# jandrewrfarrell/RUFUS

Hardware: AMD Instinct MI355X
Metric: reads/sec through k-mer count+filter at k=25 (higher is better)
Workload: dtype u64; 1 GPU; synthetic 30x WGS trio (BASELINE configs[2]): genome 3100000000 bp, 620000000/620000000/620000000 x 150 bp reads per sample, on each of 1 GPU(s) 19 resident blocks of the subject (92 GB of packed reads in HBM, generated on the device in 3.3 s), 1000 SNVs, seed 12345, k=25, -s 8G -L 2, MinCov 5, MaxHashDepth 1200, MinQ 15, thresh 1; 2 minimizer-shard pass(es) per step (per-shard (pos,key)-sorted re; parallelism=read-block shard x1, mutant_kmers=24567, pulled_pairs=11560, passes=2, hbm_total=309220868096, hbm_free_at_start=308400881664, resident_read_bytes=92219805240, read_blocks=compact, run_map_budget_bytes=39836680704, checked=False, hbm_mapped_bytes=271656681472

## Files before the change

### include/rufus_hip.h

```cpp
#ifndef RUFUS_HIP_H
#define RUFUS_HIP_H

#include <stddef.h>
#include <stdint.h>

#ifdef __cplusplus
extern "C" {
#endif

#define RFX_OK 0
#define RFX_E_NODEVICE (-1)
#define RFX_E_INVAL (-2)
#define RFX_E_NOMEM (-3)
#define RFX_E_FULL (-4)
#define RFX_E_HIP (-5)
#define RFX_E_MIXEDCASE (-6)
#define RFX_E_RANGE (-7)
#define RFX_E_FORMAT (-8)

#define RFX_HISTO_BINS 10002

typedef struct rfx_ctx rfx_ctx;
typedef struct rfx_reads rfx_reads;
typedef struct rfx_table rfx_table;
// ... 166 lines not shown
const uint64_t* rfx_records_dev_pos(const rfx_records*);
int rfx_records_histo(const rfx_records*, uint64_t* histo );
int rfx_records_verify(const rfx_records*, uint32_t min_count, uint32_t max_count, uint64_t out[4]);
int rfx_records_checksum(const rfx_records*, uint64_t out[2]);
void rfx_records_free(rfx_records*);

int rfx_merge_unique(rfx_ctx*, const rfx_records* const* files, int n_files, uint32_t min_count, uint64_t* keys_out,
                     uint32_t* counts_out, uint64_t cap, uint64_t* n_out);
int rfx_query(const rfx_records* db, const uint64_t* keys, uint64_t n, uint32_t* counts_out);
int rfx_unique_to_subject(rfx_ctx*, const rfx_records* subject, const rfx_records* const* others, int n_others,
                          uint32_t min_count, uint32_t min_cov, uint32_t max_cov, uint64_t* keys_out,
                          uint32_t* counts_out, uint64_t cap, uint64_t* n_out);
rfx_records* rfx_records_subtract(rfx_ctx*, const rfx_records* a, const rfx_records* const* others, int n_others,
                                  uint32_t min_count, uint32_t max_count);

typedef struct rfx_binned rfx_binned;
typedef struct rfx_candidates rfx_candidates;
rfx_binned* rfx_count_finish_binned(rfx_table*, uint64_t lower, uint64_t upper, uint64_t* histo );
uint64_t rfx_binned_size(const rfx_binned*);
int rfx_binned_bits(const rfx_binned*);
void rfx_binned_free(rfx_binned*);
rfx_candidates* rfx_binned_strike(rfx_ctx*, rfx_binned* subject, const rfx_binned* control, uint32_t min_count,
                                  uint32_t max_count);
int rfx_candidates_strike(rfx_candidates*, const rfx_binned* control);
uint64_t rfx_candidates_size(const rfx_candidates*);
int rfx_candidates_get(const rfx_candidates*, uint64_t* keys_out);
int rfx_candidates_get_counts(const rfx_candidates*, uint32_t* counts_out);
int rfx_candidates_strike_records(rfx_candidates*, const rfx_records* exclude);
void rfx_candidates_free(rfx_candidates*);
int rfx_binned_get(const rfx_binned*, uint64_t* keys_out, uint32_t* counts_out, uint32_t* bins_out, uint64_t* at_out,
                   uint64_t cap, uint64_t* n_out);
int rfx_binned_checksum(const rfx_binned*, uint64_t out[2]);
int rfx_binned_verify(const rfx_binned*, uint64_t lower, uint64_t upper, uint64_t out[5]);
int rfx_binned_query(const rfx_binned*, const uint64_t* canonical_keys, uint64_t n, uint32_t* counts_out);
const uint64_t* rfx_binned_dev_keys(const rfx_binned*);
const uint32_t* rfx_binned_dev_counts(const rfx_binned*);

rfx_set* rfx_set_build(rfx_ctx*, const uint64_t* fwd_keys, uint64_t n, int k);
uint64_t rfx_set_size(const rfx_set*);
void rfx_set_free(rfx_set*);
int rfx_filter(rfx_set*, const rfx_reads*, int thresh, int last_base_skipped, uint32_t* hits_out,
               uint64_t* hitmask_out, uint64_t* n_hit_reads);
int rfx_filter_many(rfx_set*, const rfx_reads* const* blocks, int n, int thresh, int last_base_skipped,
                    uint64_t* const* hitmask_out, uint64_t* n_hit_reads);

#define RFX_SELECT_READS 0
// ... 32 lines not shown
```

### profiles/summarize_pmc.py

```python
#!/usr/bin/env python3
import collections
import csv
import json
import re
import sys


NOT_CHAIN = frozenset((
    "k_synth_reads", "k_copy16",
    "k_flag_absent", "k_flag_absent_tiled", "k_fa_bounds", "k_flag_gather", "k_flag_range", "k_flag_rank", "k_flag_present",
    "k_compact_count", "k_compact_scatter", "k_scan_u64", "k_query", "k_strike_bins", "k_strike_cands",
    "k_strike_query", "k_binned_sizes", "k_binned_scan", "k_binned_gather", "k_binned_checksum", "k_binned_verify", "k_binned_query",
    "k_filter", "k_filter_q", "k_filter_p", "k_filter_fast", "k_filter_big", "k_hits_mask", "k_mask_count", "k_set_bitmap",
    "k_set_bitmap_big", "k_set_bitmap_q", "k_set_bitmap_p",
    "k_set_insert", "k_set_bitmap_packed", "k_records_checksum", "k_records_verify", "k_check_sorted",
    "k_parse_records", "k_format_records", "k_txt_count", "k_txt_lines", "k_txt_reads", "k_txt_pack", "k_txt_nth", "k_bgzf_inflate", "k_reads_tile_count", "k_reads_tile_table", "k_reads_tile", "k_select_words", "k_select_table", "k_select_copy", "k_gather_sizes", "k_gather_table", "k_gather_copy", "k_compute_pos", "k_annotate", "k_overlap_pool", "k_overlap_score",
    "k_model_colsum", "k_model_dist", "k_model_rowtot", "k_model_sum", "k_model_terms", "k_model_weights",
))
CHAIN_KNOWN = frozenset((
    "k_msp_part1", "k_msp_replay", "k_msp_count", "k_col_sums", "k_bin_group_sums", "k_bin_offsets", "k_scan_tail", "k_scan_sums",
    "k_scan_apply", "k_part2", "k_flag_if_gt", "k_slice_tag", "k_bin_hist", "k_bin_hist_stamp", "k_bin_hist_multi", "k_msp_leaf",
    "k_surv_place", "k_surv_hist", "k_surv_sort", "k_histo_bins", "k_histo_staged", "k_bin_count", "k_part1", "k_leaf", "k_leaf_compact", "k_bin_scatter",
    "k_tmp_start", "k_split_bins", "k_coarse_counts", "k_histo", "k_count_reads", "k_count_pairs", "k_table_pairs", "k_tile_count",
    "k_tile_scan", "k_tile_emit",
))


def kname(s):
    m = re.search(r"(k_[a-z0-9_]+|__amd_rocclr_[A-Za-z]+)", s)
    return m.group(1) if m else s[:40]


def load(path, counter):
    agg = collections.defaultdict(lambda: [0, 0.0])
# ... 44 lines not shown
```

### rufus_amd/capi.py

```python
from __future__ import annotations

import ctypes as C
import os
import sys

import numpy as np

_HERE = os.path.dirname(os.path.abspath(__file__))
LIB_PATH = os.environ.get("RFX_LIB") or os.path.join(_HERE, "librufus_hip.so")

HISTO_BINS = 10002
PACK_COUNT, PACK_FILTER = 1, 2
COUNT_AUTO, COUNT_TABLE, COUNT_P2L, COUNT_MSP = 0, 1, 2, 3
E_FULL, E_RANGE, E_MIXEDCASE = -4, -7, -6
E_INVAL, E_FORMAT = -2, -8
SELECT_READS, SELECT_PAIRS = 0, 1

u8p, u32p, u64p = C.POINTER(C.c_uint8), C.POINTER(C.c_uint32), C.POINTER(C.c_uint64)

SIGNATURES = {
    "rfx_version": (C.c_char_p, []),
    "rfx_strerror": (C.c_char_p, [C.c_int]),
    "rfx_last_error": (C.c_char_p, []),
    "rfx_jf_matrix": (C.c_int, [C.c_int, C.c_int, u64p]),
# ... 8 lines not shown
    "rfx_open": (C.c_void_p, [C.c_int, C.c_size_t]),
    "rfx_close": (None, [C.c_void_p]),
    "rfx_sync": (C.c_int, [C.c_void_p]),
    "rfx_host_alloc": (C.c_void_p, [C.c_size_t]),
    "rfx_host_alloc_lazy": (C.c_void_p, [C.c_size_t]),
    "rfx_host_pin": (C.c_int, [C.c_void_p]),
    "rfx_host_cpus": (C.c_uint, []),
    "rfx_host_free": (None, [C.c_void_p]),
    "rfx_stream": (C.c_void_p, [C.c_void_p]),
    "rfx_mem_stats": (C.c_int, [C.c_void_p, u64p, u64p, u64p]),
    "rfx_memcpy_dev": (C.c_int, [C.c_void_p, C.c_void_p, C.c_void_p, C.c_size_t]),
    "rfx_prof_enable": (C.c_int, [C.c_void_p, C.c_int]),
    "rfx_prof_filter": (C.c_int, [C.c_void_p, C.c_char_p]),
    "rfx_prof_reset": (C.c_int, [C.c_void_p]),
    "rfx_prof_query": (C.c_int, [C.c_void_p, C.c_char_p, C.POINTER(C.c_double), u64p]),
    "rfx_prof_names": (C.c_int, [C.c_void_p, C.c_char_p, C.c_size_t]),
    "rfx_reads_device_bytes": (C.c_uint64, [C.c_void_p]),
    "rfx_records_subtract": (C.c_void_p, [C.c_void_p, C.c_void_p, C.POINTER(C.c_void_p), C.c_int, C.c_uint32, C.c_uint32]),
    "rfx_count_finish_binned": (C.c_void_p, [C.c_void_p, C.c_uint64, C.c_uint64, u64p]),
    "rfx_binned_size": (C.c_uint64, [C.c_void_p]),
    "rfx_binned_bits": (C.c_int, [C.c_void_p]),
    "rfx_binned_free": (None, [C.c_void_p]),
    "rfx_binned_strike": (C.c_void_p, [C.c_void_p, C.c_void_p, C.c_void_p, C.c_uint32, C.c_uint32]),
    "rfx_candidates_strike": (C.c_int, [C.c_void_p, C.c_void_p]),
    "rfx_candidates_size": (C.c_uint64, [C.c_void_p]),
    "rfx_candidates_get": (C.c_int, [C.c_void_p, u64p]),
    "rfx_candidates_free": (None, [C.c_void_p]),
    "rfx_candidates_get_counts": (C.c_int, [C.c_void_p, u32p]),
    "rfx_candidates_strike_records": (C.c_int, [C.c_void_p, C.c_void_p]),
    "rfx_binned_get": (C.c_int, [C.c_void_p, u64p, u32p, u32p, u64p, C.c_uint64, u64p]),
    "rfx_binned_checksum": (C.c_int, [C.c_void_p, u64p]),
    "rfx_binned_verify": (C.c_int, [C.c_void_p, C.c_uint64, C.c_uint64, u64p]),
    "rfx_binned_query": (C.c_int, [C.c_void_p, u64p, C.c_uint64, u32p]),
    "rfx_binned_dev_keys": (C.c_void_p, [C.c_void_p]),
    "rfx_binned_dev_counts": (C.c_void_p, [C.c_void_p]),
    "rfx_reads_upload": (C.c_void_p, [C.c_void_p, u64p, u32p, u32p, u32p, u32p, C.c_uint32]),
    "rfx_reads_free": (None, [C.c_void_p]),
    "rfx_reads_count": (C.c_uint32, [C.c_void_p]),
    "rfx_reads_bases": (C.c_uint64, [C.c_void_p]),
    "rfx_reads_words": (C.c_uint64, [C.c_void_p]),
    "rfx_reads_get": (C.c_int, [C.c_void_p, u64p, u32p, u32p, u32p, u32p]),
    "rfx_tile_plan": (C.c_int, [C.c_uint64, C.c_int, C.c_uint32, u64p, u32p]),
    "rfx_reads_tile": (C.c_void_p, [C.c_void_p, C.c_void_p, C.c_int, C.c_uint32]),
    "rfx_reads_select": (C.c_void_p, [C.c_void_p, C.c_void_p, u64p, C.c_int]),
    "rfx_reads_origin": (C.c_int, [C.c_void_p, u32p, u32p]),
    "rfx_filter_pull": (C.c_void_p, [C.c_void_p, C.POINTER(C.c_void_p), C.c_int, C.c_int, C.c_int, C.c_int, C.POINTER(u64p), u64p]),
# ... 825 lines not shown
        return k[k != np.uint64(0xFFFFFFFFFFFFFFFF)]

    def counts(self, raw_keys=None) -> np.ndarray:
        c = np.zeros(len(self), np.uint32)
        _check(lib().rfx_candidates_get_counts(self._h, _p(c, u32p)), "rfx_candidates_get_counts")
        k = self._raw_keys() if raw_keys is None else raw_keys
        return c[k != np.uint64(0xFFFFFFFFFFFFFFFF)]

    def keys_counts(self):
        k = self._raw_keys()
        return k[k != np.uint64(0xFFFFFFFFFFFFFFFF)], self.counts(k)

    def free(self):
        if self._h:
            lib().rfx_candidates_free(self._h)
            self._h = None


def binned_strike(ctx: Context, subject: Binned, control, min_count: int = 0, max_count: int = 0xFFFFFFFF) -> Candidates:
    return Candidates(ctx, lib().rfx_binned_strike(ctx._h, subject._h, control._h if control is not None else None,
                                                   min_count, max_count))


OVL_SAM, OVL_CONTIG, OVL_REGION = 0, 1, 2


def overlap_score(ctx: Context, a: bytes, cands, min_pct: float, min_ovl: int, variant: int = OVL_SAM) -> np.ndarray:
    nb = len(cands)
    arr = (C.c_char_p * max(nb, 1))(*cands)
    lens = (C.c_int * max(nb, 1))(*[len(x) for x in cands])
    out = np.zeros((max(nb, 1), 5), dtype=np.int32)
    _check(lib().rfx_overlap_score(ctx._h, a, len(a), arr, lens, nb, min_pct, min_ovl, variant,
                                   out.ctypes.data_as(C.POINTER(C.c_int))), "rfx_overlap_score")
    return out[:nb]


def model_residuals(ctx: Context, histo, cands, log_resid: bool, inflection: int, max_copy: int = 5) -> np.ndarray:
    histo = np.ascontiguousarray(histo, dtype=np.int64)
    cands = np.ascontiguousarray(cands, dtype=np.float64).reshape(-1, 5)
    out = np.zeros(len(cands), dtype=np.float64)
    _check(lib().rfx_model_residuals(ctx._h, _p(histo, C.POINTER(C.c_int64)), len(histo), cands.ctypes.data, len(cands),
                                     int(bool(log_resid)), inflection, max_copy, _p(out, C.POINTER(C.c_double))),
           "rfx_model_residuals")
    return out


# ... 71 lines not shown
```

### rufus_amd/csrc/rfx_api.hip

```cpp
#include <algorithm>
#include <condition_variable>
#include <mutex>
#include <cstdio>
#include <cstdlib>
#include <cstring>
#include <sys/mman.h>

#include <atomic>
#include <cerrno>
#include <chrono>
#include <queue>
#include <thread>
#include <vector>

#include <unistd.h>

#include "rfx_internal.h"

namespace {

thread_local char g_err[512] = "";

int hip_fail(hipError_t e, const char* what) {
  snprintf(g_err, sizeof g_err, "%s: %s", what, hipGetErrorString(e));
// ... 2882 lines not shown
void rfx_binned_free(rfx_binned* b) {
  if (!b) return;
  (void)hipSetDevice(b->ctx->device);
  leaf_stage_free(b->ctx, &b->st);
  dfree(b->ctx, b->bin_at);
  delete b;
}

rfx_candidates* rfx_binned_strike(rfx_ctx* c, rfx_binned* subject, const rfx_binned* control, uint32_t min_count,
                                  uint32_t max_count) {
  if (!c || !subject || subject->ctx != c || (control && (control->ctx != c || control->k != subject->k))) {
    snprintf(g_err, sizeof g_err, "rfx_binned_strike: bad argument");
    return nullptr;
  }
  (void)hipSetDevice(c->device);
  const rfxk::binned_view S = binned_view_of(subject), C = binned_view_of(control);
  uint64_t cap = std::max<uint64_t>(1u << 16, subject->n / 256);
  if (!control) cap = std::max<uint64_t>(cap, subject->n / 4);
  for (int attempt = 0; attempt < 2; ++attempt) {
    cap = std::min<uint64_t>(std::max<uint64_t>(cap, 1), 0xFFFFFFFFull);
    uint64_t* keys = (uint64_t*)dmalloc(c, cap * 8);
    uint32_t* bins = (uint32_t*)dmalloc(c, cap * 4);
    uint32_t* counts = (uint32_t*)dmalloc(c, cap * 4);
    uint32_t* d_n = (uint32_t*)dmalloc(c, 4);
    auto drop = [&] { dfree(c, keys); dfree(c, bins); dfree(c, counts); dfree(c, d_n); };
    if (!keys || !bins || !counts || !d_n) { drop(); snprintf(g_err, sizeof g_err, "rfx_binned_strike: out of device memory"); return nullptr; }
    hipError_t e = hipMemsetAsync(d_n, 0, 4, c->stream);
    uint32_t n = 0;
    if (e == hipSuccess) {
      rfxk::strike_bins(c, S, C, min_count, max_count, keys, bins, counts, (uint32_t)cap, d_n);
      e = queue_read(c, &n, d_n, 4);
    }
    if (e == hipSuccess) e = ctx_sync(c);
    if (e != hipSuccess) { hip_fail(e, "rfx_binned_strike"); (void)ctx_sync(c); drop(); return nullptr; }
    dfree(c, d_n);
    if (n > cap) {
      dfree(c, keys);
      dfree(c, bins);
      dfree(c, counts);
      cap = n;
      continue;
    }
    rfx_candidates* r = new rfx_candidates();
    r->ctx = c;
    r->k = subject->k;
    r->bits = subject->bits;
    r->keys = keys;
    r->bins = bins;
    r->counts = counts;
    r->n = n;
    return r;
  }
  snprintf(g_err, sizeof g_err, "rfx_binned_strike: the candidate list did not converge (internal error)");
  return nullptr;
}

int rfx_candidates_strike(rfx_candidates* a, const rfx_binned* control) {
  if (!a || !control || a->ctx != control->ctx || a->k != control->k) return RFX_E_INVAL;
  rfx_ctx* c = a->ctx;
  (void)hipSetDevice(c->device);
  rfxk::strike_cands(c, a->keys, a->bins, a->n, a->bits, binned_view_of(control));
  HIPCHK(ctx_sync(c));
  return RFX_OK;
}

uint64_t rfx_candidates_size(const rfx_candidates* a) { return a ? a->n : 0; }
int rfx_candidates_get(const rfx_candidates* a, uint64_t* keys_out) {
  if (!a || (a->n && !keys_out)) return RFX_E_INVAL;
  if (!a->n) return RFX_OK;
  (void)hipSetDevice(a->ctx->device);
  HIPCHK(ctx_sync(a->ctx));
  HIPCHK(hipMemcpy(keys_out, a->keys, (size_t)a->n * 8, hipMemcpyDeviceToHost));
  return RFX_OK;
}
int rfx_candidates_get_counts(const rfx_candidates* a, uint32_t* counts_out) {
  if (!a || (a->n && !counts_out)) return RFX_E_INVAL;
  if (!a->n) return RFX_OK;
// ... 1531 lines not shown
```

### rufus_amd/csrc/rfx_internal.h

```cpp
#pragma once
#include <hip/hip_runtime.h>
#include <stdint.h>

#include <atomic>
#include <map>
#include <string>
#include <vector>

#include "../../include/rufus_hip.h"

#define RFX_EMPTY 0xFFFFFFFFFFFFFFFFull
#define RFX_TILE 1024u
#define RFX_TABLE_MARGIN 65536u
#define RFX_PROBE_LIMIT 2048u

struct rfx_prof_span {
  std::string name;
  hipEvent_t e0, e1;
};
struct rfx_prof_acc {
  double ms = 0;
  uint64_t launches = 0;
};

// ... 9 lines not shown
  int device = 0;
  hipStream_t stream = nullptr;
  hipStream_t aux = nullptr;
  size_t budget = 0, used = 0;
  int n_cu = 256;
  bool prof = false;
  std::string prof_filter;
  std::vector<rfx_prof_span> spans;
  std::vector<hipEvent_t> free_events;
  std::map<std::string, rfx_prof_acc> acc;
  std::map<void*, size_t> allocs;
  std::multimap<size_t, void*> pool;
  char* arena = nullptr;
  size_t arena_reserved = 0, arena_mapped = 0, arena_gran = 0;
  std::vector<void*> arena_handles;
  std::map<size_t, size_t> arena_free;
  bool arena_off = false;
  size_t peak_used = 0;
  std::vector<int> peer_devices;
  uint32_t lds_opt_in = 0;
  hipError_t launch_error = hipSuccess;
  std::vector<struct rfx_table*> pend_tables;
  double msp_surv_frac[2] = {0, 0};
  std::map<uint64_t, double> msp_surv_by_size;
  char* pin = nullptr;
  size_t pin_cap = 0, pin_used = 0;
  uint8_t* load_pin[3] = {nullptr, nullptr, nullptr};
  size_t load_pin_bytes = 0;
  struct pin_read { void* dst; size_t off, n; };
  std::vector<pin_read> pin_reads;
  std::map<std::pair<int, uint64_t>, rfx_hash_consts> consts;
  std::map<int, std::vector<uint64_t>> std_cols;
};

struct rfx_table_stats {
  unsigned long long distinct;
  unsigned int max_disp;
  unsigned int overflow;
};

struct rfx_count_ctl {
  unsigned int ticket;
  unsigned int stop;
  unsigned int lost;
  unsigned int pad;
  unsigned long long ovf_n;
// ... 313 lines not shown
  uint32_t chunk = 0, n_chunks = 0;
};
void msp_leaf(rfx_ctx*, const uint64_t* const* seg_inst, const uint64_t* const* seg_bs, int nseg,
              const uint64_t* inst0, const uint64_t* bs0, uint32_t P, int k, int canonical, const uint64_t* lut,
              int ntab, int sel_bits, int shift1, uint64_t pos_lo, uint64_t pos_hi, uint64_t lower, uint64_t upper,
              uint64_t* out_w, uint32_t* out_c, uint32_t* cur, uint32_t cap, unsigned int* flag, unsigned int* err,
              unsigned int* stage_short ,
              int geo ,
              const uint32_t* const* seg_ext, const uint32_t* ext0 , const msp_stage& st,
              uint32_t launch , uint32_t grid ,
              uint2* bin_at = nullptr );
struct binned_view {
  const uint64_t* keys = nullptr;
  uint32_t* counts = nullptr;
  const uint32_t* fill = nullptr;
  const uint2* bin_at = nullptr;
  uint32_t chunk = 0, n_chunks = 0, bin_lo = 0, bin_hi = 0;
  int bits = 0;
};
uint32_t msp_leaf_chunk_room(int geo, uint32_t chunk);
uint32_t msp_leaf_chunk_kept(uint32_t chunk);
void histo_staged(rfx_ctx*, const msp_stage&, unsigned long long* d_histo, unsigned long long* d_total);
void strike_bins(rfx_ctx*, const binned_view& S, const binned_view& C, uint32_t lo, uint32_t hi, uint64_t* out_k, uint32_t* out_b,
                 uint32_t* out_c, uint32_t cap, uint32_t* out_n);
void strike_cands(rfx_ctx*, uint64_t* keys, const uint32_t* bins, uint32_t n, int bits, const binned_view& C);
void binned_offsets(rfx_ctx*, const binned_view&, unsigned long long* d_offs);
void binned_gather(rfx_ctx*, const binned_view&, const unsigned long long* d_offs, uint64_t n, uint64_t* keys_out,
                   uint32_t* counts_out, uint32_t* bins_out, uint64_t* at_out);
void binned_checksum(rfx_ctx*, const msp_stage&, unsigned long long* d_out );
void binned_verify(rfx_ctx*, const binned_view&, int k, int canonical, uint64_t lower, uint64_t upper,
                   unsigned long long* d_out);
void binned_query(rfx_ctx*, const binned_view&, int k, int canonical, const uint64_t* qkeys, uint64_t nq, uint32_t* out);
void msp_leaf_plan(rfx_ctx*, uint32_t P, int geo, uint64_t n_records, uint64_t est_survivors, uint32_t extra, uint32_t* grid,
                   uint32_t* chunk, uint32_t* n_chunks);
void surv_hist(rfx_ctx*, const uint64_t* buf_a, const uint32_t* coarse_cur, uint32_t cap_a, uint32_t P2, int shift2,
               uint64_t* fine_tot, int rec_mode = 0 , int k = 0,
               uint64_t n_hint = 0);
void flag_if_gt(rfx_ctx*, const uint64_t* d_value, uint64_t limit, unsigned int* d_flag);
void histo_bins(rfx_ctx*, const uint32_t* counts, const uint32_t* coarse_cur, uint32_t cap, unsigned long long* d_histo);
void surv_sort(rfx_ctx*, const uint64_t* bw, const uint32_t* bc, const uint64_t* bs, uint32_t P, int bin_shift,
               const uint64_t* lut_inv, int ntab, int sel_bits, uint64_t* out_keys, uint32_t* out_counts,
               uint64_t* out_pos);
void tmp_start(rfx_ctx*, const uint64_t* const* seg_bs, int nseg, uint32_t P, uint64_t* out );
void leaf(rfx_ctx*, const uint64_t* const* seg_inst, const uint64_t* const* seg_bs, int nseg, const uint64_t* inst0,
          const uint64_t* bs0, uint32_t P, const rfx_ord_cfg&, uint64_t lower, uint64_t upper,
          const uint64_t* tmp_start, uint64_t* tmp_w, uint32_t* tmp_counts, uint64_t* n_surv, unsigned int* err);
void split_bins(rfx_ctx*, uint64_t* bs, uint32_t P, uint64_t n_own, uint64_t* bs2);
// ... 55 lines not shown
```

### rufus_amd/csrc/rfx_msp.hip

```cpp
#include <algorithm>
#include <type_traits>

#include "rfx_devutil.h"
#include "rfx_internal.h"

#ifdef RFX_TIMING
__device__ unsigned long long g_tm[2048][32];
#define TM_ROW g_tm[blockIdx.x & 2047u]
#define TM_DECL unsigned long long tm_prev = __builtin_amdgcn_s_memtime()
#define TM(i) do { if (threadIdx.x == 0) { const unsigned long long tm_now = __builtin_amdgcn_s_memtime(); atomicAdd(&TM_ROW[i], tm_now - tm_prev); tm_prev = tm_now; } } while (0)
extern "C" int rfx_debug_timing(unsigned long long* out, int reset) {
  static unsigned long long h[2048][32];
  if (out) {
    if (hipMemcpyFromSymbol(h, HIP_SYMBOL(g_tm), sizeof(g_tm)) != hipSuccess) return -1;
    for (int i = 0; i < 32; ++i) {
      out[i] = 0;
      for (int w = 0; w < 2048; ++w) out[i] += h[w][i];
    }
  }
  if (reset) {
    void* p = nullptr;
    if (hipGetSymbolAddress(&p, HIP_SYMBOL(g_tm)) != hipSuccess || hipMemset(p, 0, sizeof(g_tm)) != hipSuccess) return -1;
  }
  return 0;
// ... 1328 lines not shown
                                            uint32_t* __restrict__ out_n) {
  const unsigned long long m = __ballot(surv);
  if (!m) return;
  const uint32_t lane = threadIdx.x & 63u, leader = (uint32_t)__ffsll(m) - 1u;
  uint32_t base = 0;
  if (lane == leader) base = atomicAdd(out_n, (uint32_t)__popcll(m));
  base = __shfl(base, (int)leader, 64);
  if (surv) {
    const uint32_t at = base + (uint32_t)__popcll(m & ((1ull << lane) - 1ull));
    if (at < cap) {
      out_k[at] = key;
      out_b[at] = bin;
      out_c[at] = count;
    }
  }
}

constexpr int SB_BLK = 128, SB_SET_LOG2 = 11, SB_SET = 1 << SB_SET_LOG2, SB_TILE = SB_SET / 2;
__device__ __forceinline__ uint32_t sb_hash(uint64_t key) { return (uint32_t)((key * 0x9E3779B97F4A7C15ull) >> 40); }

__global__ __launch_bounds__(SB_BLK) void k_strike_bins(const rfxk::binned_view S, const rfxk::binned_view C, int ubits, uint32_t u_lo,
                                                        uint32_t u_hi, uint32_t lo, uint32_t hi, uint64_t* __restrict__ out_k,
                                                        uint32_t* __restrict__ out_b, uint32_t* __restrict__ out_c, uint32_t cap,
                                                        uint32_t* __restrict__ out_n) {
  __shared__ unsigned long long s_set[SB_SET];
  const int ds = S.bits - ubits, dc = C.bin_at ? C.bits - ubits : 0;
  for (uint32_t u = u_lo + blockIdx.x; u < u_hi; u += gridDim.x) {
    uint32_t n_s = 0, n_c = 0;
    const uint32_t s0 = u << ds, s1 = (u + 1u) << ds, c0 = u << dc, c1 = C.bin_at ? (u + 1u) << dc : c0;
    const uint4 ms = binned_marks(S, s0), mc = binned_marks(C, c0);
    binned_range(S, s0, s1, ms, [&](uint32_t, size_t, uint32_t o, uint32_t e) { n_s += e - o; });
    if (!n_s) continue;
    binned_range(C, c0, c1, mc, [&](uint32_t, size_t, uint32_t o, uint32_t e) { n_c += e - o; });
    const uint32_t tiles = n_c ? (n_c + SB_TILE - 1u) / SB_TILE : 1u;
    const bool single = tiles == 1u;
    for (uint32_t t = 0; t < tiles; ++t) {
      const uint32_t t0 = t * SB_TILE, t1 = min(t0 + (uint32_t)SB_TILE, n_c);
      uint32_t lg = 8;
      while ((1u << lg) < 2u * (t1 - t0)) ++lg;
      const uint32_t mask = (1u << lg) - 1u;
      for (uint32_t i = threadIdx.x; i <= mask; i += SB_BLK) s_set[i] = RFX_EMPTY;
      __syncthreads();
      if (t1 > t0) {
        uint32_t idx0 = 0;
        binned_range(C, c0, c1, mc, [&](uint32_t, size_t first, uint32_t o, uint32_t e) {
            const uint32_t from = max(idx0, t0), to = min(idx0 + (e - o), t1);
            for (uint32_t i = from + threadIdx.x; i < to; i += SB_BLK) {
              const unsigned long long key = C.keys[first + o + (i - idx0)];
              uint32_t h = sb_hash(key) & mask;
              for (;;) {
// ... 23 lines not shown
                  if (v == key) drop = true;
                  if (v == key || v == RFX_EMPTY) break;
                  h = (h + 1u) & mask;
                }
              }
              if (drop) {
                c = 0;
                if (!single) S.counts[first + i] = 0;
              }
            }
            if (single) cand_append(c != 0, key, b, c, out_k, out_b, out_c, cap, out_n);
          }
        });
      __syncthreads();
    }
    if (!single)
      binned_range(S, s0, s1, ms, [&](uint32_t b, size_t first, uint32_t o, uint32_t e) {
          for (uint32_t i0 = o; i0 < e; i0 += SB_BLK) {
            const uint32_t i = i0 + threadIdx.x;
            const uint32_t c = i < e ? S.counts[first + i] : 0u;
            cand_append(c != 0, c ? S.keys[first + i] : 0ull, b, c, out_k, out_b, out_c, cap, out_n);
          }
        });
  }
}

__global__ __launch_bounds__(256) void k_strike_cands(uint64_t* __restrict__ keys, const uint32_t* __restrict__ bins, uint32_t n,
                                                      int bits, const rfxk::binned_view C) {
  const uint32_t lane = threadIdx.x & 63u, wave = (blockIdx.x * 256u + threadIdx.x) >> 6, n_waves = gridDim.x * 4u;
  for (uint32_t i = wave; i < n; i += n_waves) {
    const uint64_t key = keys[i];
    if (key == RFX_EMPTY) continue;
    const uint32_t sb = bins[i];
    const uint32_t b0 = C.bits >= bits ? sb << (C.bits - bits) : sb >> (bits - C.bits);
    const uint32_t b1 = C.bits >= bits ? (sb + 1u) << (C.bits - bits) : b0 + 1u;
    bool found = false;
    for (uint32_t b = b0; b < b1; ++b)
      binned_segments(C, b, [&](size_t first, uint32_t o, uint32_t e) {
        for (uint32_t j = o + lane; j < e; j += 64u) found |= C.keys[first + j] == key;
      });
    if (__ballot(found) && lane == 0) keys[i] = RFX_EMPTY;
  }
}

__global__ __launch_bounds__(256) void k_histo_staged(const uint32_t* __restrict__ counts, const uint32_t* __restrict__ fill,
                                                       const uint32_t* __restrict__ more, uint32_t CH, uint32_t n_chunks,
// ... 307 lines not shown
      if (geo) RFX_MSP_LEAF(false, 1);
      else RFX_MSP_LEAF(false, 0);
    }
#undef RFX_MSP_LEAF
  }
  if (!bin_at) {
    rfx_span sp(c, "k_surv_place");
    const uint32_t pg = std::min<uint32_t>(st.n_chunks, (uint32_t)c->n_cu * (uint32_t)std::max(1, 160 * 1024 / (16 * 1024 + SP_N * 12 + 2048)));
    hipLaunchKernelGGL(k_surv_place, dim3(pg), dim3(SP_BLK), 0, c->stream, st.keys, st.counts, st.chunk, st.fill, more, grid,
                       st.n_chunks, lut, ntab, sel_bits, shift1, pos_lo, pos_hi, out_w, out_c, cur, cap, flag);
  }
}

uint32_t msp_leaf_chunk_room(int geo, uint32_t chunk) { return chunk - MSP_LEAF_PASS_MAX(geo); }
uint32_t msp_leaf_chunk_kept(uint32_t chunk) { return chunk >= 16384u ? 65536u : chunk; }

void histo_staged(rfx_ctx* c, const msp_stage& st, unsigned long long* d_histo, unsigned long long* d_total) {
  rfx_span sp(c, "k_histo");
  const uint32_t grid = std::max<uint32_t>(1, std::min<uint32_t>(st.n_chunks, (uint32_t)c->n_cu * 4));
  hipLaunchKernelGGL(k_histo_staged, dim3(grid), dim3(256), 0, c->stream, st.counts, st.fill, st.more, st.chunk, st.n_chunks,
                     d_histo, d_total);
}

void strike_bins(rfx_ctx* c, const binned_view& S, const binned_view& C, uint32_t lo, uint32_t hi, uint64_t* out_k,
                 uint32_t* out_b, uint32_t* out_c, uint32_t cap, uint32_t* out_n) {
  rfx_span sp(c, "k_strike_bins");
  const int ubits = C.bin_at ? std::min(S.bits, C.bits) : S.bits;
  const int ds = S.bits - ubits;
  const uint32_t u_lo = S.bin_lo >> ds, u_hi = (uint32_t)((((uint64_t)S.bin_hi + (1u << ds) - 1)) >> ds);
  if (u_hi <= u_lo) return;
  const uint32_t grid = std::min<uint32_t>(u_hi - u_lo, (uint32_t)c->n_cu * 10);
  hipLaunchKernelGGL(k_strike_bins, dim3(grid), dim3(SB_BLK), 0, c->stream, S, C, ubits, u_lo, u_hi, lo, hi, out_k, out_b, out_c,
                     cap, out_n);
}

void strike_cands(rfx_ctx* c, uint64_t* keys, const uint32_t* bins, uint32_t n, int bits, const binned_view& C) {
  if (!n) return;
  rfx_span sp(c, "k_strike_cands");
  const uint32_t grid = std::min<uint32_t>((n + 3) / 4, (uint32_t)c->n_cu * 8);
  hipLaunchKernelGGL(k_strike_cands, dim3(grid), dim3(256), 0, c->stream, keys, bins, n, bits, C);
}

void binned_offsets(rfx_ctx* c, const binned_view& v, unsigned long long* d_offs) {
  rfx_span sp(c, "k_binned_get");
  const uint32_t nb = v.bin_hi - v.bin_lo;
  if (nb) {
    const uint32_t grid = std::max<uint32_t>(1, std::min<uint32_t>((nb + 255u) / 256u, (uint32_t)c->n_cu * 8));
    hipLaunchKernelGGL(k_binned_sizes, dim3(grid), dim3(256), 0, c->stream, v, d_offs);
  }
  hipLaunchKernelGGL(k_binned_scan, dim3(1), dim3(BSC_BLK), 0, c->stream, d_offs, nb);
}

void binned_gather(rfx_ctx* c, const binned_view& v, const unsigned long long* d_offs, uint64_t n, uint64_t* keys_out,
                   uint32_t* counts_out, uint32_t* bins_out, uint64_t* at_out) {
  const uint32_t nb = v.bin_hi - v.bin_lo;
  if (!nb || !n) return;
// ... 67 lines not shown
```

Measured before the change: 1.108 billion reads/s.

## Strike trio bins with a wave-per-unit kernel and defer oversized units to block kernel

Adds k_strike_wave, in which each 64-lane wave handles one strike unit entirely in registers and a per-wave LDS hash set. Units whose subject or control size or segment count exceeds the caps are deferred to a list, and k_strike_bins then processes only those deferred units. The aim is to cut per-unit block-level overhead and raise parallelism on the many small units of the trio strike. The cost is a second launch, the atomic defer list and added complexity. Env knobs and a stats API are added for tuning.

New measurement: 1.128 billion reads/s, median of 6. 1.02x the previous value.

```diff
diff --git a/include/rufus_hip.h b/include/rufus_hip.h
--- a/include/rufus_hip.h
+++ b/include/rufus_hip.h
@@ -212,6 +212,7 @@
 void rfx_binned_free(rfx_binned*);
 rfx_candidates* rfx_binned_strike(rfx_ctx*, rfx_binned* subject, const rfx_binned* control, uint32_t min_count,
                                   uint32_t max_count);
+int rfx_binned_strike_stats(const rfx_ctx*, uint64_t out[2]);
 int rfx_candidates_strike(rfx_candidates*, const rfx_binned* control);
 uint64_t rfx_candidates_size(const rfx_candidates*);
 int rfx_candidates_get(const rfx_candidates*, uint64_t* keys_out);
diff --git a/profiles/strike_wave.py b/profiles/strike_wave.py
--- /dev/null
+++ b/profiles/strike_wave.py
@@ -0,0 +1,164 @@
+import argparse
+import csv
+import filecmp
+import glob
+import json
+import os
+import shutil
+import subprocess
+import sys
+import tempfile
+
+ROOT = os.path.dirname(os.path.dirname(os.path.abspath(__file__)))
+K, JF_SIZE, LOWER, MIN_COV, MAX_DEPTH, MIN_Q, THRESH, READ_LEN, SEED, COVERAGE = 25, 8 << 30, 2, 5, 1200, 15, 1, 150, 12345, 30
+
+
+def stats_row(genome, passes):
+    sys.path.insert(0, ROOT)
+    from rufus_amd import capi, wgs
+    seen = []
+    inner = capi.binned_strike
+
+    def strike(ctx, *a, **kw):
+        r = inner(ctx, *a, **kw)
+        seen.append(capi.binned_strike_stats(ctx))
+        return r
+    capi.binned_strike = strike
+    n_pairs = genome * COVERAGE // (2 * READ_LEN)
+    sys_ = [capi.Synth.sample(genome, w, n_snv=max(20, min(1000, genome // 3_000_000)), seed=SEED, read_len=READ_LEN) for w in range(3)]
+    with capi.Context(0) as ctx:
+        samples = [wgs.make_sample(ctx, sy, n_pairs, 1 << 24, MIN_Q, want_good=(i == 0), compact=True) for i, sy in enumerate(sys_)]
+        trio = wgs.WgsTrio(ctx, K, JF_SIZE, LOWER, MIN_COV, MAX_DEPTH, THRESH, passes=passes)
+        trio.masks_are_views = True
+        res = trio.run(samples)
+        units, deferred = sum(s["units"] for s in seen), sum(s["deferred"] for s in seen)
+        print(f"stats     genome {genome} passes {passes}: " + "  ".join(f"strike {i}: {s['units']} units, {s['deferred']} deferred"
+                                                                          for i, s in enumerate(seen))
+              + f"   deferred share {100.0 * deferred / max(units, 1):.4f} %   mutant_kmers {res['n_mutant']}", flush=True)
+        trio.close()
+        for s in samples:
+            for b in s:
+                b.free()
+
+
+def run(args, cwd, limit, env=None, stdout=subprocess.PIPE):
+    p = subprocess.run(args, cwd=cwd, stdout=stdout, stderr=subprocess.PIPE, timeout=limit, env=dict(os.environ, **(env or {})))
+    if p.returncode != 0:
+        sys.stdout.write(f"FAILED rc {p.returncode}: {' '.join(args)} (in {cwd})\n" + p.stderr.decode()[-2000:] + "\n")
+        raise SystemExit(1)
+    return p.stdout.decode() if stdout == subprocess.PIPE else ""
+
+
+def bench_line(tree, extra=(), limit=420):
+    return json.loads(run([sys.executable, "bench.py"] + list(extra), tree, limit).strip().splitlines()[-1])
+
+
+def strike_ms(tree, label, work):
+    d = os.path.join(work, "trace_" + label)
+    run(["rocprofv3", "--kernel-trace", "--output-format", "csv", "-d", d, "-o", "t", "--", sys.executable, "bench.py", "--steps", "1",
+         "--warmup", "2", "--inner"], tree, 420)
+    src = glob.glob(os.path.join(d, "**", "t_kernel_trace.csv"), recursive=True)[0]
+    dst = os.path.join(work, label + "_stats.csv")
+    meta = json.loads(run([sys.executable, os.path.join(ROOT, "profiles", "summarize_trace.py"), src, dst], ROOT, 120).strip().splitlines()[-1])
+    out = {}
+    for r in csv.DictReader(open(dst)):
+        for name in ("k_strike_wave", "k_strike_bins", "k_strike_cands"):
+            if name + "<" in r["Name"] or name + "(" in r["Name"]:
+                c, t = out.get(name, (0, 0.0))
+                out[name] = (c + int(r["Calls"]), t + float(r["TotalDurationNs"]) / 1e6)
+    shutil.rmtree(d, ignore_errors=True)
+    total = sum(t for n, (c, t) in out.items() if n != "k_strike_cands")
+    print(f"kernel    {label:10s} " + "  ".join(f"{n} {t:.3f} ms in {c} launches" for n, (c, t) in sorted(out.items()))
+          + f"   strike per step {total:.3f} ms   all kernels of the step {meta['kernel_ms']:.1f} ms", flush=True)
+    return total, out
+
+
+def main():
+    ap = argparse.ArgumentParser()
+    ap.add_argument("--parent", default=None)
+    ap.add_argument("--variant", action="append", default=[], help="LABEL=TREE")
+    ap.add_argument("--runs", type=int, default=3)
+    ap.add_argument("--only", default="headline,kernel,pmc,stats,same")
+    ap.add_argument("--pmc-round", default="r13")
+    ap.add_argument("--commit", default="Trio strike: k_strike_wave takes the plain units, on top of 4e421fc")
+    ap.add_argument("--stats-row", action="store_true", help="(internal) the child of the `stats` row")
+    ap.add_argument("--genome", type=int, default=1_000_000_000)
+    ap.add_argument("--passes", type=int, default=2)
+    args = ap.parse_args()
+    if args.stats_row:
+        return stats_row(args.genome, args.passes)
+    only = set(args.only.split(","))
+    parent = os.path.abspath(args.parent) if args.parent else None
+    variants = [(v.split("=", 1)[0], os.path.abspath(v.split("=", 1)[1])) for v in args.variant]
+    work = tempfile.mkdtemp(prefix="strike_wave_")
+    try:
+        if "headline" in only:
+            ms = {"parent": [], "new": []}
+            facts = {}
+            for i in range(args.runs):
+                for label, tree in (("parent", parent), ("new", ROOT)):
+                    ln = bench_line(tree)
+                    ms[label].append(ln["ms_per_step"])
+                    c = ln["config"]
+                    facts[label] = (c["mutant_kmers"], c["pulled_pairs"], c["hbm_peak_bytes"])
+                    print(f"headline  {label:6s} run {i}: ms_per_step {ln['ms_per_step']:9.3f}   value {ln['value']:.4e} reads/s   mutant_kmers "
+                          f"{c['mutant_kmers']}  pulled_pairs {c['pulled_pairs']}  hbm_peak_bytes {c['hbm_peak_bytes']}", flush=True)
+            mean = {k: sum(v) / len(v) for k, v in ms.items()}
+            spread = {k: max(v) - min(v) for k, v in ms.items()}
+            gap = mean["parent"] - mean["new"]
+            below = max(ms["new"]) < min(ms["parent"])
+            enough = gap >= 5 * max(spread.values())
+            print(f"headline  means: parent {mean['parent']:.3f}  new {mean['new']:.3f}  gap {gap:.3f} ms ({100 * gap / mean['parent']:.2f} %)   "
+                  f"spreads: parent {spread['parent']:.3f}  new {spread['new']:.3f}   every new run below every parent run: {below}   "
+                  f"gap >= 5 x larger spread ({5 * max(spread.values()):.3f}): {enough}   -> {'MET' if below and enough else 'NOT MET'}")
+            print(f"headline  results: mutant_kmers / pulled_pairs equal: {facts['parent'][:2] == facts['new'][:2]}   hbm_peak_bytes new "
+                  f"{facts['new'][2]} vs parent {facts['parent'][2]}: {'not above' if facts['new'][2] <= facts['parent'][2] else 'ABOVE'}", flush=True)
+        totals = {}
+        if "kernel" in only:
+            for label, tree in ([("parent", parent)] if parent else []) + [("new", ROOT)] + variants:
+                totals[label] = strike_ms(tree, label, work)
+        if "stats" in only:
+            sys.stdout.write(run([sys.executable, os.path.abspath(__file__), "--stats-row", "--genome", str(args.genome), "--passes",
+                                  str(args.passes)], ROOT, 300))
+            for label, tree in variants:
+                out = run([sys.executable, os.path.join(tree, "profiles", "strike_wave.py"), "--stats-row", "--genome", str(args.genome),
+                           "--passes", str(args.passes)], tree, 300)
+                sys.stdout.write(out.replace("stats    ", f"stats {label}", 1))
+            sys.stdout.flush()
+        if "pmc" in only:
+            for ctr, tag in (("FETCH_SIZE", "f"), ("WRITE_SIZE", "w")):
+                run(["rocprofv3", "--pmc", ctr, "--output-format", "csv", "-d", os.path.join(work, "pmc_" + tag), "-o", tag, "--",
+                     sys.executable, "bench.py", "--steps", "1", "--warmup", "0", "--inner"], ROOT, 900)
+            f = glob.glob(os.path.join(work, "pmc_f", "**", "f_counter_collection.csv"), recursive=True)[0]
+            w = glob.glob(os.path.join(work, "pmc_w", "**", "w_counter_collection.csv"), recursive=True)[0]
+            js = os.path.join(ROOT, "profiles", f"{args.pmc_round}_pmc_wgs.json")
+            summary = run([sys.executable, os.path.join(ROOT, "profiles", "summarize_pmc.py"), f, w, js, "3", "3100000000"], ROOT, 300,
+                          env={"RFX_COMMIT": args.commit})
+            open(os.path.join(ROOT, "profiles", f"{args.pmc_round}_pmc_summary_wgs.txt"), "w").write(summary)
+            pmc = json.load(open(js))
+            old = json.load(open(os.path.join(ROOT, "profiles", "r12_pmc_wgs.json")))
+            for name in ("k_strike_wave", "k_strike_bins"):
+                if name in pmc:
+                    print(f"pmc       new    {name}: {pmc[name]['hbm_bytes_per_launch'] / 1e9:.2f} GB per launch, {pmc[name]['launches']} launches", flush=True)
+            print(f"pmc       parent k_strike_bins: {old['k_strike_bins']['hbm_bytes_per_launch'] / 1e9:.2f} GB per launch (r12_pmc_wgs.json)")
+            if "new" in totals and "parent" in totals:
+                nb = sum(pmc[n]["hbm_bytes_per_launch"] * pmc[n]["launches"] for n in ("k_strike_wave", "k_strike_bins") if n in pmc)
+                ob = old["k_strike_bins"]["hbm_bytes_per_launch"] * old["k_strike_bins"]["launches"]
+                print(f"pmc       effective: parent {ob / totals['parent'][0] / 1e9:.2f} TB/s   new {nb / totals['new'][0] / 1e9:.2f} TB/s", flush=True)
+        if "same" in only:
+            dirs = {}
+            for label, tree in (("parent", parent), ("new", ROOT)):
+                dirs[label] = os.path.join(work, "dump_" + label)
+                ln = bench_line(tree, ["--genome", "300000000", "--dump-outputs", dirs[label]])
+                print(f"same      {label:6s} --genome 300000000: mutant_kmers {ln['config']['mutant_kmers']}  pulled_pairs {ln['config']['pulled_pairs']}", flush=True)
+            for name in ("mutant_keys", "histograms", "records_per_sample", "hit_reads"):
+                a, b = (os.path.join(dirs[x], name + ".npy") for x in ("parent", "new"))
+                same = filecmp.cmp(a, b, shallow=False)
+                print(f"same      {name}.npy: {'byte-identical' if same else 'DIFFERENT'} ({os.path.getsize(b)} bytes)", flush=True)
+                if not same:
+                    raise SystemExit(1)
+    finally:
+        shutil.rmtree(work, ignore_errors=True)
+
+
+main()
diff --git a/profiles/summarize_pmc.py b/profiles/summarize_pmc.py
--- a/profiles/summarize_pmc.py
+++ b/profiles/summarize_pmc.py
@@ -9,7 +9,7 @@
 NOT_CHAIN = frozenset((
     "k_synth_reads", "k_copy16",
     "k_flag_absent", "k_flag_absent_tiled", "k_fa_bounds", "k_flag_gather", "k_flag_range", "k_flag_rank", "k_flag_present",
-    "k_compact_count", "k_compact_scatter", "k_scan_u64", "k_query", "k_strike_bins", "k_strike_cands",
+    "k_compact_count", "k_compact_scatter", "k_scan_u64", "k_query", "k_strike_bins", "k_strike_wave", "k_strike_cands",
     "k_strike_query", "k_binned_sizes", "k_binned_scan", "k_binned_gather", "k_binned_checksum", "k_binned_verify", "k_binned_query",
     "k_filter", "k_filter_q", "k_filter_p", "k_filter_fast", "k_filter_big", "k_hits_mask", "k_mask_count", "k_set_bitmap",
     "k_set_bitmap_big", "k_set_bitmap_q", "k_set_bitmap_p",
diff --git a/rufus_amd/capi.py b/rufus_amd/capi.py
--- a/rufus_amd/capi.py
+++ b/rufus_amd/capi.py
@@ -54,6 +54,7 @@
     "rfx_binned_bits": (C.c_int, [C.c_void_p]),
     "rfx_binned_free": (None, [C.c_void_p]),
     "rfx_binned_strike": (C.c_void_p, [C.c_void_p, C.c_void_p, C.c_void_p, C.c_uint32, C.c_uint32]),
+    "rfx_binned_strike_stats": (C.c_int, [C.c_void_p, u64p]),
     "rfx_candidates_strike": (C.c_int, [C.c_void_p, C.c_void_p]),
     "rfx_candidates_size": (C.c_uint64, [C.c_void_p]),
     "rfx_candidates_get": (C.c_int, [C.c_void_p, u64p]),
@@ -925,6 +926,12 @@
                                                    min_count, max_count))
 
 
+def binned_strike_stats(ctx: Context) -> dict:
+    o = np.zeros(2, dtype=np.uint64)
+    _check(lib().rfx_binned_strike_stats(ctx._h, _p(o, u64p)), "rfx_binned_strike_stats")
+    return {"units": int(o[0]), "deferred": int(o[1])}
+
+
 OVL_SAM, OVL_CONTIG, OVL_REGION = 0, 1, 2
 
 
diff --git a/rufus_amd/csrc/rfx_api.hip b/rufus_amd/csrc/rfx_api.hip
--- a/rufus_amd/csrc/rfx_api.hip
+++ b/rufus_amd/csrc/rfx_api.hip
@@ -2928,17 +2928,20 @@
     uint64_t* keys = (uint64_t*)dmalloc(c, cap * 8);
     uint32_t* bins = (uint32_t*)dmalloc(c, cap * 4);
     uint32_t* counts = (uint32_t*)dmalloc(c, cap * 4);
-    uint32_t* d_n = (uint32_t*)dmalloc(c, 4);
+    const uint32_t n_units = rfxk::strike_units(S, C);
+    uint32_t* d_n = (uint32_t*)dmalloc(c, ((size_t)n_units + 2) * 4);
     auto drop = [&] { dfree(c, keys); dfree(c, bins); dfree(c, counts); dfree(c, d_n); };
     if (!keys || !bins || !counts || !d_n) { drop(); snprintf(g_err, sizeof g_err, "rfx_binned_strike: out of device memory"); return nullptr; }
-    hipError_t e = hipMemsetAsync(d_n, 0, 4, c->stream);
-    uint32_t n = 0;
+    hipError_t e = hipMemsetAsync(d_n, 0, 8, c->stream);
+    uint32_t got[2] = {0, 0};
     if (e == hipSuccess) {
-      rfxk::strike_bins(c, S, C, min_count, max_count, keys, bins, counts, (uint32_t)cap, d_n);
-      e = queue_read(c, &n, d_n, 4);
+      rfxk::strike_bins(c, S, C, min_count, max_count, keys, bins, counts, (uint32_t)cap, d_n, d_n + 2, d_n + 1);
+      e = queue_read(c, got, d_n, 8);
     }
     if (e == hipSuccess) e = ctx_sync(c);
     if (e != hipSuccess) { hip_fail(e, "rfx_binned_strike"); (void)ctx_sync(c); drop(); return nullptr; }
+    const uint32_t n = got[0];
+    c->strike_deferred = c->strike_by_wave ? got[1] : c->strike_units;
     dfree(c, d_n);
     if (n > cap) {
       dfree(c, keys);
@@ -2959,6 +2962,13 @@
   }
   snprintf(g_err, sizeof g_err, "rfx_binned_strike: the candidate list did not converge (internal error)");
   return nullptr;
+}
+
+int rfx_binned_strike_stats(const rfx_ctx* c, uint64_t out[2]) {
+  if (!c || !out) return RFX_E_INVAL;
+  out[0] = c->strike_units;
+  out[1] = c->strike_deferred;
+  return RFX_OK;
 }
 
 int rfx_candidates_strike(rfx_candidates* a, const rfx_binned* control) {
diff --git a/rufus_amd/csrc/rfx_internal.h b/rufus_amd/csrc/rfx_internal.h
--- a/rufus_amd/csrc/rfx_internal.h
+++ b/rufus_amd/csrc/rfx_internal.h
@@ -55,6 +55,8 @@
   hipError_t launch_error = hipSuccess;
   std::vector<struct rfx_table*> pend_tables;
   double msp_surv_frac[2] = {0, 0};
+  uint64_t strike_units = 0, strike_deferred = 0;
+  bool strike_by_wave = false;
   std::map<uint64_t, double> msp_surv_by_size;
   char* pin = nullptr;
   size_t pin_cap = 0, pin_used = 0;
@@ -414,7 +416,8 @@
 uint32_t msp_leaf_chunk_kept(uint32_t chunk);
 void histo_staged(rfx_ctx*, const msp_stage&, unsigned long long* d_histo, unsigned long long* d_total);
 void strike_bins(rfx_ctx*, const binned_view& S, const binned_view& C, uint32_t lo, uint32_t hi, uint64_t* out_k, uint32_t* out_b,
-                 uint32_t* out_c, uint32_t cap, uint32_t* out_n);
+                 uint32_t* out_c, uint32_t cap, uint32_t* out_n, uint32_t* defer, uint32_t* n_defer);
+uint32_t strike_units(const binned_view& S, const binned_view& C);
 void strike_cands(rfx_ctx*, uint64_t* keys, const uint32_t* bins, uint32_t n, int bits, const binned_view& C);
 void binned_offsets(rfx_ctx*, const binned_view&, unsigned long long* d_offs);
 void binned_gather(rfx_ctx*, const binned_view&, const unsigned long long* d_offs, uint64_t n, uint64_t* keys_out,
diff --git a/rufus_amd/csrc/rfx_msp.hip b/rufus_amd/csrc/rfx_msp.hip
--- a/rufus_amd/csrc/rfx_msp.hip
+++ b/rufus_amd/csrc/rfx_msp.hip
@@ -1374,10 +1374,14 @@
 __global__ __launch_bounds__(SB_BLK) void k_strike_bins(const rfxk::binned_view S, const rfxk::binned_view C, int ubits, uint32_t u_lo,
                                                         uint32_t u_hi, uint32_t lo, uint32_t hi, uint64_t* __restrict__ out_k,
                                                         uint32_t* __restrict__ out_b, uint32_t* __restrict__ out_c, uint32_t cap,
-                                                        uint32_t* __restrict__ out_n) {
+                                                        uint32_t* __restrict__ out_n, const uint32_t* __restrict__ units,
+                                                        const uint32_t* __restrict__ n_units) {
   __shared__ unsigned long long s_set[SB_SET];
   const int ds = S.bits - ubits, dc = C.bin_at ? C.bits - ubits : 0;
-  for (uint32_t u = u_lo + blockIdx.x; u < u_hi; u += gridDim.x) {
+  const uint32_t n_u = units ? min(*n_units, u_hi - u_lo) : u_hi - u_lo;
+  for (uint32_t ui = blockIdx.x; ui < n_u; ui += gridDim.x) {
+    const uint32_t u = units ? units[ui] : u_lo + ui;
+    if (u < u_lo || u >= u_hi) continue;
     uint32_t n_s = 0, n_c = 0;
     const uint32_t s0 = u << ds, s1 = (u + 1u) << ds, c0 = u << dc, c1 = C.bin_at ? (u + 1u) << dc : c0;
     const uint4 ms = binned_marks(S, s0), mc = binned_marks(C, c0);
@@ -1447,6 +1451,165 @@
             cand_append(c != 0, c ? S.keys[first + i] : 0ull, b, c, out_k, out_b, out_c, cap, out_n);
           }
         });
+  }
+}
+
+#ifndef RFX_SW_SET_LOG2
+#define RFX_SW_SET_LOG2 10
+#endif
+#ifndef RFX_SW_PER
+#define RFX_SW_PER 12
+#endif
+constexpr int SW_BLK = 256, SW_WAVES = SW_BLK / 64, SW_SET_LOG2 = RFX_SW_SET_LOG2, SW_SET = 1 << SW_SET_LOG2, SW_PER = RFX_SW_PER;
+constexpr uint32_t SW_CAP_C = 3 * SW_SET / 4 < 64 * SW_PER ? 3 * SW_SET / 4 : 64 * SW_PER, SW_CAP_S = 64 * SW_PER;
+
+__device__ __forceinline__ void sw_sync() {
+  __builtin_amdgcn_fence(__ATOMIC_ACQ_REL, "wavefront");
+  __builtin_amdgcn_wave_barrier();
+}
+
+__device__ __forceinline__ uint4 sw_uniform(const uint4 m) {
+  return make_uint4(__builtin_amdgcn_readfirstlane(m.x), __builtin_amdgcn_readfirstlane(m.y), __builtin_amdgcn_readfirstlane(m.z),
+                    __builtin_amdgcn_readfirstlane(m.w));
+}
+constexpr int SW_SEGS = 2;
+struct sw_side {
+  size_t base[SW_SEGS];
+  uint32_t start[SW_SEGS], bin[SW_SEGS];
+  uint32_t n = 0, segs = 0;
+  __device__ __forceinline__ sw_side() {
+#pragma unroll
+    for (int q = 0; q < SW_SEGS; ++q) {
+      base[q] = 0;
+      start[q] = ~0u;
+      bin[q] = 0;
+    }
+  }
+  __device__ __forceinline__ void add(uint32_t b, size_t first, uint32_t o, uint32_t e) {
+#pragma unroll
+    for (int q = 0; q < SW_SEGS; ++q)
+      if (segs == (uint32_t)q) {
+        base[q] = first + o - n;
+        start[q] = n;
+        bin[q] = b;
+      }
+    ++segs;
+    n += e - o;
+  }
+  __device__ __forceinline__ void uniform() {
+#pragma unroll
+    for (int q = 0; q < SW_SEGS; ++q) {
+      base[q] = (size_t)__builtin_amdgcn_readfirstlane((uint32_t)base[q]) |
+                (size_t)__builtin_amdgcn_readfirstlane((uint32_t)(base[q] >> 32)) << 32;
+      start[q] = __builtin_amdgcn_readfirstlane(start[q]);
+      bin[q] = __builtin_amdgcn_readfirstlane(bin[q]);
+    }
+    n = __builtin_amdgcn_readfirstlane(n);
+    segs = __builtin_amdgcn_readfirstlane(segs);
+  }
+  __device__ __forceinline__ size_t at(uint32_t j, uint32_t* b) const {
+    static_assert(SW_SEGS == 2, "one select");
+    j = min(j, n - 1u);
+    const bool second = j >= start[1];
+    *b = second ? bin[1] : bin[0];
+    return (second ? base[1] : base[0]) + j;
+  }
+};
+
+template <bool FINE>
+__global__ __launch_bounds__(SW_BLK) void k_strike_wave(const rfxk::binned_view S, const rfxk::binned_view C, int ubits, uint32_t u_lo,
+                                                        uint32_t u_hi, uint32_t lo, uint32_t hi, uint32_t cap_c, uint32_t cap_s,
+                                                        uint64_t* __restrict__ out_k, uint32_t* __restrict__ out_b,
+                                                        uint32_t* __restrict__ out_c, uint32_t cap, uint32_t* __restrict__ out_n,
+                                                        uint32_t* __restrict__ defer, uint32_t* __restrict__ n_defer) {
+  __shared__ unsigned long long s_sets[SW_WAVES][SW_SET];
+  constexpr uint32_t mask = SW_SET - 1u;
+  const uint32_t lane = threadIdx.x & 63u, n_waves = gridDim.x * SW_WAVES;
+  unsigned long long* const set = s_sets[threadIdx.x >> 6];
+  const int ds = S.bits - ubits, dc = C.bin_at ? C.bits - ubits : 0;
+  cap_c = min(cap_c, SW_CAP_C);
+  cap_s = min(cap_s, SW_CAP_S);
+  for (uint32_t i = lane; i < (uint32_t)SW_SET; i += 64u) set[i] = RFX_EMPTY;
+  sw_sync();
+  uint32_t u = u_lo + blockIdx.x * SW_WAVES + (threadIdx.x >> 6);
+  if (u >= u_hi) return;
+  uint4 ms = binned_marks(S, u << ds), mc = binned_marks(C, u << dc);
+  for (bool more = true; more; u += n_waves) {
+    const uint32_t s0 = u << ds, s1 = (u + 1u) << ds, c0 = u << dc, c1 = C.bin_at ? (u + 1u) << dc : c0;
+    const uint4 ms_u = sw_uniform(ms), mc_u = sw_uniform(mc);
+    more = u_hi - u > n_waves;
+    sw_side ss, cs;
+    binned_range(S, s0, s1, ms_u, [&](uint32_t b, size_t first, uint32_t o, uint32_t e) { ss.add(b, first, o, e); });
+    if (ss.n) binned_range(C, c0, c1, mc_u, [&](uint32_t b, size_t first, uint32_t o, uint32_t e) { cs.add(b, first, o, e); });
+    ss.uniform();
+    cs.uniform();
+    const uint32_t n_s = ss.n, n_c = cs.n;
+    const bool plain = n_c <= cap_c && n_s <= cap_s && ss.segs <= (uint32_t)SW_SEGS && cs.segs <= (uint32_t)SW_SEGS;
+    const uint32_t rows_c = plain ? (n_c + 63u) >> 6 : 0u, rows_s = plain ? (n_s + 63u) >> 6 : 0u;
+    unsigned long long ck[SW_PER], sk[SW_PER];
+    uint32_t sc[SW_PER], sb[SW_PER];
+#pragma unroll
+    for (int p = 0; p < SW_PER; ++p)
+      if ((uint32_t)p < rows_c) {
+        uint32_t b;
+        ck[p] = C.keys[cs.at(lane + 64u * (uint32_t)p, &b)];
+      }
+#pragma unroll
+    for (int p = 0; p < SW_PER; ++p)
+      if ((uint32_t)p < rows_s) {
+        const size_t a = ss.at(lane + 64u * (uint32_t)p, &sb[p]);
+        sk[p] = S.keys[a];
+        sc[p] = S.counts[a];
+      }
+    if (more) {
+      ms = binned_marks(S, (u + n_waves) << ds);
+      mc = binned_marks(C, (u + n_waves) << dc);
+    }
+    if (!n_s) continue;
+    if (!plain) {
+      if (lane == 0) defer[atomicAdd(n_defer, 1u)] = u;
+      continue;
+    }
+    uint32_t slot[SW_PER];
+#pragma unroll
+    for (int p = 0; p < SW_PER; ++p) {
+      slot[p] = ~0u;
+      if ((uint32_t)p >= rows_c) continue;
+      if (lane + 64u * (uint32_t)p < n_c) {
+        const unsigned long long key = ck[p];
+        uint32_t h = sb_hash(key) & mask;
+        for (uint32_t t = 0; t < (uint32_t)SW_SET; ++t) {
+          const unsigned long long old = atomicCAS(&set[h], (unsigned long long)RFX_EMPTY, key);
+          if (old == RFX_EMPTY) slot[p] = h;
+          if (old == RFX_EMPTY || old == key) break;
+          h = (h + 1u) & mask;
+        }
+      }
+    }
+    sw_sync();
+#pragma unroll
+    for (int p = 0; p < SW_PER; ++p) {
+      if ((uint32_t)p >= rows_s) continue;
+      const unsigned long long key = sk[p];
+      uint32_t c = lane + 64u * (uint32_t)p < n_s ? sc[p] : 0u;
+      if (c && (c < lo || c > hi)) c = 0;
+      if (c && n_c) {
+        uint32_t h = sb_hash(key) & mask;
+        for (uint32_t t = 0; t < (uint32_t)SW_SET; ++t) {
+          const unsigned long long v = set[h];
+          if (v == key) c = 0;
+          if (v == key || v == RFX_EMPTY) break;
+          h = (h + 1u) & mask;
+        }
+      }
+      cand_append(c != 0, key, FINE ? sb[p] : u, c, out_k, out_b, out_c, cap, out_n);
+    }
+    sw_sync();
+#pragma unroll
+    for (int p = 0; p < SW_PER; ++p) {
+      if ((uint32_t)p < rows_c && slot[p] != ~0u) set[slot[p]] = RFX_EMPTY;
+    }
+    sw_sync();
   }
 }
 
@@ -1800,16 +1963,55 @@
                      d_histo, d_total);
 }
 
+uint32_t strike_units(const binned_view& S, const binned_view& C) {
+  const int ds = S.bits - (C.bin_at ? std::min(S.bits, C.bits) : S.bits);
+  const uint32_t u_lo = S.bin_lo >> ds, u_hi = (uint32_t)((((uint64_t)S.bin_hi + (1u << ds) - 1)) >> ds);
+  return u_hi > u_lo ? u_hi - u_lo : 0;
+}
+
 void strike_bins(rfx_ctx* c, const binned_view& S, const binned_view& C, uint32_t lo, uint32_t hi, uint64_t* out_k,
-                 uint32_t* out_b, uint32_t* out_c, uint32_t cap, uint32_t* out_n) {
-  rfx_span sp(c, "k_strike_bins");
+                 uint32_t* out_b, uint32_t* out_c, uint32_t cap, uint32_t* out_n, uint32_t* defer, uint32_t* n_defer) {
   const int ubits = C.bin_at ? std::min(S.bits, C.bits) : S.bits;
   const int ds = S.bits - ubits;
   const uint32_t u_lo = S.bin_lo >> ds, u_hi = (uint32_t)((((uint64_t)S.bin_hi + (1u << ds) - 1)) >> ds);
+  c->strike_units = strike_units(S, C);
+  c->strike_by_wave = false;
   if (u_hi <= u_lo) return;
   const uint32_t grid = std::min<uint32_t>(u_hi - u_lo, (uint32_t)c->n_cu * 10);
+  const char* const wg = getenv("RFX_STRIKE_WG");
+  if ((wg && atoi(wg)) || !defer || !n_defer) {
+    rfx_span sp(c, "k_strike_bins");
+    hipLaunchKernelGGL(k_strike_bins, dim3(grid), dim3(SB_BLK), 0, c->stream, S, C, ubits, u_lo, u_hi, lo, hi, out_k, out_b, out_c,
+                       cap, out_n, (const uint32_t*)nullptr, (const uint32_t*)nullptr);
+    return;
+  }
+  uint32_t cap_c = SW_CAP_C, cap_s = SW_CAP_S;
+  if (const char* e = getenv("RFX_STRIKE_WAVE_CAP")) {
+    unsigned a = 0, b = 0;
+    if (sscanf(e, "%u,%u", &a, &b) == 2) {
+      cap_c = std::min<uint32_t>(cap_c, a);
+      cap_s = std::min<uint32_t>(cap_s, b);
+    }
+  }
+  int per_cu = 0;
+  const hipError_t oe = ds ? hipOccupancyMaxActiveBlocksPerMultiprocessor(&per_cu, k_strike_wave<true>, SW_BLK, 0)
+                           : hipOccupancyMaxActiveBlocksPerMultiprocessor(&per_cu, k_strike_wave<false>, SW_BLK, 0);
+  if (oe != hipSuccess || per_cu < 1) per_cu = 4;
+  uint32_t wgrid = std::min<uint32_t>((u_hi - u_lo + SW_WAVES - 1) / SW_WAVES, (uint32_t)c->n_cu * (uint32_t)per_cu);
+  if (const char* e = getenv("RFX_STRIKE_WAVE_GRID")) wgrid = std::max<uint32_t>(1, std::min<uint32_t>(wgrid, (uint32_t)atoi(e)));
+  c->strike_by_wave = true;
+  {
+    rfx_span sp(c, "k_strike_wave");
+    if (ds)
+      hipLaunchKernelGGL(k_strike_wave<true>, dim3(wgrid), dim3(SW_BLK), 0, c->stream, S, C, ubits, u_lo, u_hi, lo, hi, cap_c, cap_s,
+                         out_k, out_b, out_c, cap, out_n, defer, n_defer);
+    else
+      hipLaunchKernelGGL(k_strike_wave<false>, dim3(wgrid), dim3(SW_BLK), 0, c->stream, S, C, ubits, u_lo, u_hi, lo, hi, cap_c, cap_s,
+                         out_k, out_b, out_c, cap, out_n, defer, n_defer);
+  }
+  rfx_span sp(c, "k_strike_bins");
   hipLaunchKernelGGL(k_strike_bins, dim3(grid), dim3(SB_BLK), 0, c->stream, S, C, ubits, u_lo, u_hi, lo, hi, out_k, out_b, out_c,
-                     cap, out_n);
+                     cap, out_n, (const uint32_t*)defer, (const uint32_t*)n_defer);
 }
 
 void strike_cands(rfx_ctx* c, uint64_t* keys, const uint32_t* bins, uint32_t n, int bits, const binned_view& C) {
```
